# gregorgebhardt/gym-kilobots

Measured on AMD Instinct MI355X. Metric: kilobot-steps/sec, higher is better.
Workload: dtype f32

## Files before the change

### gym_kilobots_amd/csrc/kb_common.h

```cpp
#pragma once
#include <hip/hip_runtime.h>

#include <cmath>
#include <cstdio>
#include <cstring>
#include <type_traits>

#include "kilobots_hip.h"
#include "kb_launch.h"
#include "kb_exact.h"

namespace kb {

constexpr float B2_PI = 3.14159265359f;
constexpr float B2_LINEAR_SLOP = 0.005f;
constexpr float B2_POLYGON_RADIUS = 2.0f * B2_LINEAR_SLOP;
constexpr float B2_BAUMGARTE = 0.2f;
constexpr float B2_MAX_LINEAR_CORRECTION = 0.2f;
constexpr float B2_MAX_TRANSLATION = 2.0f;
constexpr float B2_MAX_TRANSLATION_SQ = B2_MAX_TRANSLATION * B2_MAX_TRANSLATION;
constexpr float B2_MAX_ROTATION = 0.5f * B2_PI;
constexpr float B2_MAX_ROTATION_SQ = B2_MAX_ROTATION * B2_MAX_ROTATION;
constexpr float B2_EPSILON = 1.19209290e-07f;
constexpr float B2_TOI_BAUMGARTE = 0.75f;
constexpr int B2_MAX_SUBSTEPS = 8;
constexpr float B2_TIME_TO_SLEEP = 0.5f;
constexpr float B2_LINEAR_SLEEP_TOL = 0.01f;
constexpr float B2_ANGULAR_SLEEP_TOL = 2.0f / 180.0f * B2_PI;
constexpr float WORLD_SCALE = 25.0f;

constexpr float CELL_SIZE = 0.875f;
constexpr int MAX_CELLS = 8192;

constexpr unsigned KEY_WALL = 0x10000u, KEY_OBJ = 0x20000u;
constexpr int WALL_CODE = 0xFFF0;
constexpr int OBJ_CODE = 0xFFE0;
constexpr int MAXOBJ = KB_MAX_OBJECTS;
constexpr unsigned short EMPTY16 = 0xFFFFu;

#ifndef KB_KREG
#define KB_KREG 2
#endif
constexpr int MAX_BUCKETS = MAX_WAVES * BK_PER_WAVE;
constexpr int GIANT_ISLAND = 256;
constexpr int BIG_ISLAND = 16;
constexpr int KREG = KB_KREG;
#ifndef KB_NSOLVE_DIV
#define KB_NSOLVE_DIV 1
#endif
#ifndef KB_KREG_BINS
#define KB_KREG_BINS (2 * KB_NSOLVE_DIV)
#endif

enum { M_NCON = 0, M_TOTAL = 1, M_ANY = 2, M_STATUS = 3, M_MAXISL = 4, M_PROF = 5, M_XTRA = 6, M_XFILL = 7, M_WCNT = 8, M_WAKE = 32 , M_WFILL = 8 + MAX_WAVES, M_COUNT = 8 + 2 * MAX_WAVES };
static_assert(M_COUNT <= 64, "misc area");

struct Params {
    kb_buffers buf;
    const float *actions;
    const float *light_action;
    int N, NP, NB, M, E, S, gw, gh, ncell, cap, capL, n_substeps, flags, drive_mode, light_type, vel_iters, pos_iters;
    int solver_mode, toi_walls;
    float xmin, ymin, xmax, ymax, inv_cell, r_bot, im_bot, kl_bot, ka_bot, h;
    float light_radius, light_lo[2], light_hi[2], act_lo[2], act_hi[2];
    int lcount, ladim, lkind[KB_MAX_LIGHTS];
    float lradius[KB_MAX_LIGHTS], lmaxv[KB_MAX_LIGHTS];
    float llo[KB_MAX_LIGHTS][2], lhi[KB_MAX_LIGHTS][2], lalo[KB_MAX_LIGHTS][2], lahi[KB_MAX_LIGHTS][2];
    float kl_obj, ka_obj;
    float otab[KB_MAX_OBJECTS][OT_WORDS_C];
    float obody[KB_MAX_OBJECTS][BT_WORDS_C];
    int F;
    float mu_oo, mu_ow;
    int nmc;
    int lds_total;
    int nhead, hmask;
    int allow_sleep;
    float im_mode[5];
    int botlaw_off;
    int islmin_off;
    int sense_s;
    float sense_r2;
    float rr2, rw2, rw_tot;
    float toi_tt;
    float nm_bb, nm_wb;
    float y_bb, y_wb;
    int exact_div;
    const unsigned char *env_mask;
};


__device__ __forceinline__ void kb_sincosf(float xx, float &sn, float &cs) {
    const float DP1 = 0.78515625f, DP2 = 2.4187564849853515625e-4f, DP3 = 3.77489497744594108e-8f;
    const float FOPI = 1.27323954473516f;
    float x = fabsf(xx);
    int j = (int)(FOPI * x);
    float y = (float)j;
    if (j & 1) { j += 1; y += 1.0f; }
    j &= 7;
    float ssign = xx < 0.0f ? -1.0f : 1.0f, csign = 1.0f;
    if (j > 3) { ssign = -ssign; csign = -csign; j -= 4; }
    if (j > 1) csign = -csign;
    x = ((x - y * DP1) - y * DP2) - y * DP3;
    float z = x * x;
    float pc = ((2.443315711809948E-005f * z - 1.388731625493765E-003f) * z + 4.166664568298827E-002f) * z * z
               - 0.5f * z + 1.0f;
    float ps = ((-1.9515295891E-4f * z + 8.3321608736E-3f) * z - 1.6666654611E-1f) * z * x + x;
    if (j == 1 || j == 2) { sn = ssign * pc; cs = csign * ps; }
    else { sn = ssign * ps; cs = csign * pc; }
}

__device__ __forceinline__ void kb_light_circular(float sx, float sy, float lx, float ly, float R,
                                                  float &val, float &gx, float &gy) {
    float dx = -1.0f * (sx - lx), dy = -1.0f * (sy - ly);
    float n = sqrtf(dx * dx + dy * dy);
    float v = 1.0f - n / R;
    v = fmaxf(fminf(v, 1.0f), 0.0f);
    val = v * 255.0f;
    if (n > 0.0f) { dx = dx / n; dy = dy / n; }
    else { dx = 0.0f; dy = 0.0f; }
    if (n > R) { dx *= 0.0f; dy *= 0.0f; }
    gx = dx; gy = dy;
}

__device__ __forceinline__ void kb_light_single_step(const Params &p, const float *la, float h, float &lx, float &ly) {
    float ax = fminf(fmaxf(la[0], p.act_lo[0]), p.act_hi[0]);
    float ay = fminf(fmaxf(la[1], p.act_lo[1]), p.act_hi[1]);
    float nlx = lx + ax * h, nly = ly + ay * h;
    lx = fminf(fmaxf(nlx, p.light_lo[0]), p.light_hi[0]);
    ly = fminf(fmaxf(nly, p.light_lo[1]), p.light_hi[1]);
}
__device__ __forceinline__ void kb_light_general_step(const Params &p, const float *la, float h, float (&glx)[KB_MAX_LIGHTS],
                                                      float (&gly)[KB_MAX_LIGHTS], float (&glvx)[KB_MAX_LIGHTS], float (&glvy)[KB_MAX_LIGHTS]) {
    if (p.light_type == KB_LIGHT_GRADIENT) {
        const float pi = 3.14159265358979323846f;
        float ang = fminf(fmaxf(la[0], -2.0f * pi), 2.0f * pi);
        if (ang < -pi) ang += 2.0f * pi;
        if (ang > pi) ang -= 2.0f * pi;
        glx[0] = ang;
    } else {
#pragma unroll
        for (int i = 0; i < KB_MAX_LIGHTS; ++i) {
            if (i >= p.lcount) break;
            const float ax = fminf(fmaxf(la[2 * i + 0], p.lalo[i][0]), p.lahi[i][0]);
            const float ay = fminf(fmaxf(la[2 * i + 1], p.lalo[i][1]), p.lahi[i][1]);
            float nlx, nly;
            if (p.lkind[i] == KB_LIGHT_MOMENTUM) {
                float mvx = glvx[i] + ax * h, mvy = glvy[i] + ay * h;
                const float nv = sqrtf(mvx * mvx + mvy * mvy);
                if (nv > p.lmaxv[i]) { const float sc = p.lmaxv[i] / nv; mvx *= sc; mvy *= sc; }
                glvx[i] = mvx; glvy[i] = mvy;
                nlx = glx[i] + mvx * h; nly = gly[i] + mvy * h;
            } else {
                nlx = glx[i] + ax * h; nly = gly[i] + ay * h;
            }
            glx[i] = fminf(fmaxf(nlx, p.llo[i][0]), p.lhi[i][0]);
            gly[i] = fminf(fmaxf(nly, p.llo[i][1]), p.lhi[i][1]);
        }
    }
}
__device__ __forceinline__ void kb_light_general_sense(const Params &p, const float (&glx)[KB_MAX_LIGHTS], const float (&gly)[KB_MAX_LIGHTS],
                                                       float sx, float sy, float &val, float &gx, float &gy) {
    if (p.light_type == KB_LIGHT_GRADIENT) {
        float s_, c_;
        kb_sincosf(glx[0], s_, c_);
        val = c_ * sx + s_ * sy; gx = c_; gy = s_;
        return;
    }
    float vsum = 0.0f, vbest = 0.0f, bgx = 0.0f, bgy = 0.0f;
#pragma unroll
    for (int i = 0; i < KB_MAX_LIGHTS; ++i) {
        if (i >= p.lcount) break;
        float v, x, y;
        kb_light_circular(sx, sy, glx[i], gly[i], p.lradius[i], v, x, y);
        vsum = i == 0 ? v : vsum + v;
        if (i == 0 || v > vbest) { vbest = v; bgx = x; bgy = y; }
    }
    val = vsum; gx = bgx; gy = bgy;
}

__device__ __forceinline__ void kb_motor_law(int ml, int mr, float th, float h, float &vx, float &vy, float &w) {
    const float max_lin = 0.01f, max_ang = 0.5f * 3.14159265358979323846f;
    float s, c;
    kb_sincosf(th, s, c);
    if (ml && mr) {
        float lin = (float)(mr + ml) / 510.0f * max_lin;
        vx = (s * lin) * WORLD_SCALE; vy = (c * lin) * WORLD_SCALE;
        w = (float)(mr - ml) / 510.0f * max_ang;
    } else if (mr || ml) {
        float av, lx, ly = -0.009f;
        if (mr) { av = (float)mr / 255.0f * max_ang; lx = -0.013f; }
        else { av = -(float)ml / 255.0f * max_ang; lx = 0.013f; }
        float ds, dc;
        kb_sincosf(av * h, ds, dc);
        float tx = lx - (dc * lx - ds * ly), ty = ly - (ds * lx + dc * ly);
        tx *= WORLD_SCALE; ty *= WORLD_SCALE;
        float wx = c * tx - s * ty, wy = s * tx + c * ty;
        wx = wx / WORLD_SCALE / h; wy = wy / WORLD_SCALE / h;
        vx = wx * WORLD_SCALE; vy = wy * WORLD_SCALE; w = av;
    } else {
        vx = 0.0f; vy = 0.0f; w = 0.0f;
    }
}

__device__ __forceinline__ float kb_clampf(float a, float lo, float hi) { return fmaxf(lo, fminf(a, hi)); }

__device__ __forceinline__ void wave_sync() {
    __builtin_amdgcn_fence(__ATOMIC_RELEASE, "wavefront");
    __builtin_amdgcn_wave_barrier();
    __builtin_amdgcn_fence(__ATOMIC_ACQUIRE, "wavefront");
}

template <bool DS_ATOMIC = false>
__device__ __forceinline__ unsigned lds_load_relaxed(const unsigned *p_) {
    if constexpr (DS_ATOMIC) return atomicOr(const_cast<unsigned *>(p_), 0u);
    else return *reinterpret_cast<const volatile unsigned *>(p_);
}

__device__ __forceinline__ void lds_barrier() {
    asm volatile("s_waitcnt lgkmcnt(0)\n\ts_barrier" ::: "memory");
}

#define KB_DPP(v, ctrl, rows) __builtin_amdgcn_update_dpp(0, (int)(v), ctrl, rows, 0xf, true)
__device__ __forceinline__ unsigned wave_or(unsigned v) {
    v |= (unsigned)KB_DPP(v, 0x111, 0xf);
    v |= (unsigned)KB_DPP(v, 0x112, 0xf);
    v |= (unsigned)KB_DPP(v, 0x114, 0xf);
    v |= (unsigned)KB_DPP(v, 0x118, 0xf);
    v |= (unsigned)KB_DPP(v, 0x142, 0xa);
    v |= (unsigned)KB_DPP(v, 0x143, 0xc);
    return (unsigned)__builtin_amdgcn_readlane((int)v, 63);
}
__device__ __forceinline__ unsigned wave_umax(unsigned v) {
    v = max(v, (unsigned)KB_DPP(v, 0x111, 0xf));
    v = max(v, (unsigned)KB_DPP(v, 0x112, 0xf));
    v = max(v, (unsigned)KB_DPP(v, 0x114, 0xf));
    v = max(v, (unsigned)KB_DPP(v, 0x118, 0xf));
    v = max(v, (unsigned)KB_DPP(v, 0x142, 0xa));
    v = max(v, (unsigned)KB_DPP(v, 0x143, 0xc));
    return (unsigned)__builtin_amdgcn_readlane((int)v, 63);
}
__device__ __forceinline__ unsigned wave_incl_scan(unsigned v) {
    v += (unsigned)KB_DPP(v, 0x111, 0xf);
    v += (unsigned)KB_DPP(v, 0x112, 0xf);
    v += (unsigned)KB_DPP(v, 0x114, 0xf);
    v += (unsigned)KB_DPP(v, 0x118, 0xf);
    v += (unsigned)KB_DPP(v, 0x142, 0xa);
    v += (unsigned)KB_DPP(v, 0x143, 0xc);
    return v;
}

template <class AR>
__device__ __forceinline__ void wall_geom(const AR &p, int wl, float x, float y, float &dist, float &nx, float &ny) {
    switch (wl) {
    case 0: nx = 1.0f; ny = 0.0f; dist = x - p.xmin; break;
    case 1: nx = 0.0f; ny = 1.0f; dist = y - p.ymin; break;
    case 2: nx = -1.0f; ny = 0.0f; dist = p.xmax - x; break;
    default: nx = 0.0f; ny = -1.0f; dist = p.ymax - y; break;
    }
}

#ifdef KB_PROFILE
#define KB_PROF(k) misc[24 + (k)]
#define KB_STAMP(ph) do { if (tid == 0) { const unsigned t_ = (unsigned)clock64(); atomicAdd(&KB_PROF(ph), t_ - prof_t); prof_t = t_; } } while (0)
#define KB_STAMP_PRE(ph) do { if (tid == 0) { atomicAdd(&KB_PROF(ph), (unsigned)clock64() - prof_t); } } while (0)
#else
#define KB_STAMP(ph) do { } while (0)
#define KB_STAMP_PRE(ph) do { } while (0)
#endif

template <class AR>
__device__ __forceinline__ bool kb_toi_wall(const AR &p, int wl, float R, float x0, float y0, float x1, float y1, float &tout) {
    const float total = R + B2_POLYGON_RADIUS;
    const float target = fmaxf(B2_LINEAR_SLOP, total - 3.0f * B2_LINEAR_SLOP);
    const float tol = 0.25f * B2_LINEAR_SLOP;
    float nx, ny;
    auto dist_at = [&](float t) __attribute__((always_inline)) -> float {
        float dv;
        wall_geom(p, wl, (1.0f - t) * x0 + t * x1, (1.0f - t) * y0 + t * y1, dv, nx, ny);
        return dv;
    };
    float t1 = 0.0f;
    for (int iter = 0; iter < 20; ++iter) {
        const float dist = dist_at(t1);
        if (fabsf(dist) <= 0.0f) return false;
        if (fabsf(dist) < target + tol) { tout = t1; return true; }
        float t2 = 1.0f;
        for (int push = 0; push < 8; ++push) {
            float s2 = dist_at(t2);
            if (s2 > target + tol) return false;
            if (s2 > target - tol) { t1 = t2; break; }
            float s1 = dist_at(t1);
            if (s1 < target - tol) return false;
            if (s1 <= target + tol) { tout = t1; return true; }
            float a1 = t1, a2 = t2;
            for (int root = 0; root < 50; ++root) {
                const float t = (root & 1) ? a1 + (target - s1) * (a2 - a1) / (s2 - s1) : 0.5f * (a1 + a2);
                const float sv = dist_at(t);
                if (fabsf(sv - target) < tol) { t2 = t; break; }
                if (sv > target) { a1 = t; s1 = sv; } else { a2 = t; s2 = sv; }
            }
        }
    }
    return false;
}

template <class AR>
__device__ __forceinline__ bool kb_toi_no_event(const AR &p, int wl, float tt, float x0, float y0, float x1, float y1) {
    float d0, d1, nx, ny;
    wall_geom(p, wl, (1.0f - 0.0f) * x0 + 0.0f * x1, (1.0f - 0.0f) * y0 + 0.0f * y1, d0, nx, ny);
    wall_geom(p, wl, (1.0f - 1.0f) * x0 + 1.0f * x1, (1.0f - 1.0f) * y0 + 1.0f * y1, d1, nx, ny);
    return fabsf(d0) <= 0.0f || (!(fabsf(d0) < tt) && d1 > tt);
}

__device__ __forceinline__ void kb_toi_walls_body(const Params &p, float R, float im, float x0, float y0, float a0,
                                                  float &x, float &y, float &a, float &vx, float &vy, float &w) {
    const float h = p.h;
    const float total = R + B2_POLYGON_RADIUS;
    {
        const float m0 = fminf(fminf(x0 - p.xmin, p.xmax - x0), fminf(y0 - p.ymin, p.ymax - y0));
        const float m1 = fminf(fminf(x - p.xmin, p.xmax - x), fminf(y - p.ymin, p.ymax - y));
        if (m0 > total && m1 > total) return;
    }
    float alpha0 = 0.0f;
    float c0x = x0, c0y = y0, ca0 = a0, cx = x, cy = y, ca = a;
    for (int ev = 0; ev < B2_MAX_SUBSTEPS; ++ev) {
        float minAlpha = 1.0f;
#pragma unroll
        for (int wl = 0; wl < 4; ++wl) {
            float t;
            float alpha = 1.0f;
            if (kb_toi_wall(p, wl, R, c0x, c0y, cx, cy, t)) alpha = fminf(alpha0 + (1.0f - alpha0) * t, 1.0f);
            if (alpha < minAlpha) minAlpha = alpha;
        }
        if (1.0f - 10.0f * B2_EPSILON < minAlpha) break;
        const float beta = (minAlpha - alpha0) / (1.0f - alpha0);
        c0x += beta * (cx - c0x); c0y += beta * (cy - c0y); ca0 += beta * (ca - ca0);
        alpha0 = minAlpha;
        cx = c0x; cy = c0y; ca = ca0;
        bool touch[4];
        float wnx[4], wny[4];
#pragma unroll
        for (int wl = 0; wl < 4; ++wl) {
            float dist;
            wall_geom(p, wl, cx, cy, dist, wnx[wl], wny[wl]);
            touch[wl] = !(dist * dist > total * total);
            if (dist < 0.0f) { wnx[wl] = -wnx[wl]; wny[wl] = -wny[wl]; }
        }
        for (int it = 0; it < 20; ++it) {
            float minSep = 0.0f;
#pragma unroll
            for (int wl = 0; wl < 4; ++wl) {
                if (!touch[wl]) continue;
                float dist, bx, by;
                wall_geom(p, wl, cx, cy, dist, bx, by);
// ... 234 lines not shown
```

### gym_kilobots_amd/csrc/kb_regsolve_bins.inc

```
{
    constexpr int KRB = KB_KREG_BINS;
    const bool solving = (int)__builtin_amdgcn_readfirstlane(wave) < nsolve;
    unsigned ra[KRB], rb[KRB], rm[KRB];
    float racc[KRB], rnx[KRB], rny[KRB];
    const unsigned WOFF = 8u * (unsigned)(NB - 5);
    char *const velB = reinterpret_cast<char *>(vel), *const posB = reinterpret_cast<char *>(pos);
#define RB_WALL(j) (ra[j] >= WOFF)
#define RB_WALLIDX(j) ((int)((ra[j] - WOFF) >> 3))
#define RB_VEL(off) (*reinterpret_cast<float2 *>(velB + (off)))
#define RB_POS(off) (*reinterpret_cast<float2 *>(posB + (off)))
#define RB_C(j) ((int)(rm[j] & 0xFFFu))
#define RB_DEPTH(j) ((int)((rm[j] >> 12) & 0x1FFu))
#define RB_FLIP(j) (((rm[j] >> 21) & 1u) != 0u)
#define RB_ISL(j) ((int)(rm[j] >> 22))
#pragma unroll
    for (int j = 0; j < KRB; ++j) { ra[j] = 0u; rb[j] = 0u; rm[j] = 0u; racc[j] = 0.0f; rnx[j] = 1.0f; rny[j] = 0.0f; }
    unsigned long long slotLevels[KRB];
    int dlo[KRB], dhi[KRB];
#pragma unroll
    for (int j = 0; j < KRB; ++j) { slotLevels[j] = 0ull; dlo[j] = 1; dhi[j] = 0; }
    int maxD = 0;
    unsigned mycnt = 0;
    const float nm_bb = p.nm_bb, nm_wb = p.nm_wb;
#ifdef KB_SOLVER_PRIO
    __builtin_amdgcn_s_setprio(KB_SOLVER_PRIO);
#endif
    if (solving) {
        mycnt = misc[M_WCNT + wave];
        const unsigned mybase = misc[M_WFILL + wave] - mycnt;
        unsigned lk[KRB];
        unsigned lp[KRB];
        int rdepth[KRB];
        unsigned klo[KRB], khi[KRB];
#define RB_A(j) ((int)(lp[j] & 0xFFFFu))
#define RB_B(j) ((int)(lp[j] >> 16))
        {
            unsigned c_[KRB], inf_[KRB];
            bool v_[KRB], awake_[KRB];
#pragma unroll
            for (int j = 0; j < KRB; ++j) {
                const unsigned idx = lane + 64u * j;
                v_[j] = idx < mycnt;
                c_[j] = lOrder[v_[j] ? mybase + idx : 0u];
            }
#pragma unroll
            for (int j = 0; j < KRB; ++j) {
                c_[j] = v_[j] ? c_[j] : 0u;
                lp[j] = lPair[c_[j]]; inf_[j] = lInfo[c_[j]];
            }
#pragma unroll
            for (int j = 0; j < KRB; ++j) { lp[j] = v_[j] ? lp[j] : 0u; awake_[j] = true; }
            if (SLEEP) {
                unsigned root_[KRB];
#pragma unroll
                for (int j = 0; j < KRB; ++j) root_[j] = parent[lp[j] >> 16];
#pragma unroll
                for (int j = 0; j < KRB; ++j) awake_[j] = active[root_[j]] != 0;
            }
#pragma unroll
            for (int j = 0; j < KRB; ++j) {
                const unsigned cls = inf_[j] & 0x7Fu, r = (inf_[j] >> 8) & 0xFFu;
                unsigned key = cls * RK + (r < RK - 1 ? r : RK - 1);
                const bool on = v_[j] && awake_[j];
                if (!on) key = 63u;
                const unsigned bit = on ? 1u << (key & 31u) : 0u;
                klo[j] = key < 32u ? bit : 0u; khi[j] = key < 32u ? 0u : bit;
                if (on && r >= RK - 1) atomicMax(&bkMaxRank[wave * NUM_CLS + cls], r);
                lk[j] = v_[j] ? (key | (r << 8) | (c_[j] << 16) | 0x80000000u) : 0u;
                rdepth[j] = 0;
            }
        }
        unsigned long long keymask = 0ull, restmask = 0ull;
        {
            unsigned mlo = 0, mhi = 0, rlo = 0, rhi = 0;
#pragma unroll
            for (int j = 0; j < KRB; ++j) { mlo |= klo[j]; mhi |= khi[j]; if (j > 0) { rlo |= klo[j]; rhi |= khi[j]; } }
            mlo = wave_or(mlo); mhi = wave_or(mhi);
            keymask = ((unsigned long long)mhi << 32) | mlo;
            if (mycnt > 64u) { rlo = wave_or(rlo); rhi = wave_or(rhi); restmask = ((unsigned long long)rhi << 32) | rlo; }
        }
        wave_sync();
#ifdef KB_PROFILE
        if (tid == 0) { atomicAdd(&KB_PROF(8), (unsigned)__popcll(keymask)); atomicAdd(&KB_PROF(11), 1u); }
#endif
        KB_STAMP_PRE(19);
        unsigned *bodyDepth = islCnt;
        {
            char *const bdB = reinterpret_cast<char *>(bodyDepth);
#define RB_BD(off) (*reinterpret_cast<unsigned *>(bdB + (off)))
            unsigned rc[KRB], ia4[KRB], ib4[KRB];
#pragma unroll
            for (int j = 0; j < KRB; ++j) {
                const unsigned key = lk[j] & 63u, r = (lk[j] >> 8) & 0xFFu;
                const bool on = (lk[j] >> 31) != 0u && key != 63u;
                rc[j] = on ? ((key % RK) == RK - 1 ? (key | (r << 6)) : key) : 0xFFFFFFFFu;
                ib4[j] = 4u * (unsigned)RB_B(j);
                ia4[j] = RB_A(j) < WALL_CODE ? 4u * (unsigned)RB_A(j) : ib4[j];
            }
            const unsigned mrow = bkMaxRank[wave * NUM_CLS + min((int)lane, NUM_CLS - 1)];
            for (unsigned long long m_ = keymask; m_; m_ &= m_ - 1) {
                const unsigned key_ = (unsigned)__builtin_ctzll(m_);
                const bool rest_ = ((restmask >> key_) & 1ull) != 0ull;
                auto depth_round = [&](unsigned code_) __attribute__((always_inline)) {
#pragma unroll
                    for (int j = 0; j < KRB; ++j) {
                        if (j == 0 || rest_) {
                            if (rc[j] == code_) {
                                const unsigned d = max(RB_BD(ia4[j]), RB_BD(ib4[j])) + 1u;
                                rdepth[j] = (int)d;
                                RB_BD(ib4[j]) = d;
                                RB_BD(ia4[j]) = d;
                            }
                        }
                    }
                    wave_sync();
                };
                if ((key_ % RK) < RK - 1) depth_round(key_);
                else {
                    const unsigned maxr_ = (unsigned)__builtin_amdgcn_readlane((int)mrow, (int)(key_ / RK));
                    for (unsigned r_ = RK - 1; r_ <= maxr_; ++r_) depth_round(key_ | (r_ << 6));
                }
            }
#undef RB_BD
        }
#pragma unroll
        for (int j = 0; j < KRB; ++j) maxD = max(maxD, rdepth[j]);
        maxD = (int)wave_umax((unsigned)maxD);
        KB_STAMP_PRE(20);
        if (mycnt > 64u) {
            unsigned at[KRB];
#pragma unroll
            for (int j = 0; j < KRB; ++j) at[j] = 0u;
            unsigned base_ = 0;
            for (int d_ = SLEEP ? 0 : 1; d_ <= maxD; ++d_) {
#pragma unroll
                for (int j = 0; j < KRB; ++j) {
                    const bool is = (lk[j] >> 31) && rdepth[j] == d_;
                    const unsigned long long m_ = __ballot(is);
                    const unsigned mine = __builtin_amdgcn_mbcnt_hi((unsigned)(m_ >> 32), __builtin_amdgcn_mbcnt_lo((unsigned)m_, base_));
                    at[j] = is ? mine : at[j];
                    base_ += (unsigned)__popcll(m_);
                }
            }
#pragma unroll
            for (int j = 0; j < KRB; ++j)
                if (lk[j] >> 31) {
                    lOrder[mybase + at[j]] = (unsigned short)((lk[j] >> 16) & 0xFFFu);
                    lCbk[mybase + at[j]] = (unsigned short)rdepth[j];
                }
            wave_sync();
            unsigned short o_[KRB], l_[KRB];
#pragma unroll
            for (int j = 0; j < KRB; ++j) {
                const unsigned i_ = mybase + ((lk[j] >> 31) ? lane + 64u * j : 0u);
                o_[j] = lOrder[i_]; l_[j] = lCbk[i_];
            }
#pragma unroll
            for (int j = 0; j < KRB; ++j) {
                const bool v_ = (lk[j] >> 31) != 0u;
                lk[j] = v_ ? ((lk[j] & 0x8000FFFFu) | ((unsigned)o_[j] << 16)) : lk[j];
                rdepth[j] = v_ ? (int)l_[j] : rdepth[j];
            }
        }
        KB_STAMP_PRE(21);
#pragma unroll
        for (int j = 0; j < KRB; ++j) {
            const unsigned long long mine = (lk[j] >> 31) ? 1ull << min(rdepth[j], 63) : 0ull;
            const unsigned lo = wave_or((unsigned)mine), hi = wave_or((unsigned)(mine >> 32));
            slotLevels[j] = ((unsigned long long)hi << 32) | (unsigned long long)lo;
            const unsigned long long lv = slotLevels[j] >> 1;
            dlo[j] = lv ? (int)__builtin_ctzll(lv) + 1 : 1;
            dhi[j] = lv ? ((lv >> 62) ? maxD : 64 - (int)__builtin_clzll(lv)) : 0;
        }
        {
            unsigned c_[KRB], pr_[KRB], inf_[KRB], root_[KRB];
            float acc_[KRB];
            float2 pa_[KRB], pb_[KRB];
            bool v_[KRB];
#pragma unroll
            for (int j = 0; j < KRB; ++j) {
                v_[j] = (lk[j] >> 31) != 0u;
                c_[j] = v_[j] ? (lk[j] >> 16) & 0xFFFu : 0u;
                pr_[j] = lPair[c_[j]]; inf_[j] = lInfo[c_[j]]; acc_[j] = lAcc[c_[j]];
            }
#pragma unroll
            for (int j = 0; j < KRB; ++j) {
                pr_[j] = v_[j] ? pr_[j] : 0u;
                const int a = (int)(pr_[j] & 0xFFFFu), b = (int)(pr_[j] >> 16);
                pa_[j] = pos[a >= WALL_CODE ? b : a]; pb_[j] = pos[b]; root_[j] = parent[b];
            }
            bool pairOn[KRB];
            float dx[KRB], dy[KRB], dd[KRB], wnx[KRB], wny[KRB];
            bool ieee = false;
#pragma unroll
            for (int j = 0; j < KRB; ++j) {
                const int a = (int)(pr_[j] & 0xFFFFu), b = (int)(pr_[j] >> 16);
                const bool wallA = a >= WALL_CODE, flip = (inf_[j] & 0x80u) != 0u;
                ra[j] = wallA ? WOFF + 8u * (unsigned)(a - WALL_CODE) : 8u * (unsigned)a;
                rb[j] = 8u * (unsigned)b;
                racc[j] = v_[j] ? acc_[j] : 0.0f;
                rm[j] = v_[j] ? (c_[j] | ((unsigned)rdepth[j] << 12) | (flip ? 1u << 21 : 0u) | (root_[j] << 22)) : 0u;
                float dist;
                wall_geom(p, wallA ? a - WALL_CODE : 0, pb_[j].x, pb_[j].y, dist, wnx[j], wny[j]);
                if (flip) { wnx[j] = -wnx[j]; wny[j] = -wny[j]; }
                dx[j] = pb_[j].x - pa_[j].x; dy[j] = pb_[j].y - pa_[j].y;
                dd[j] = dx[j] * dx[j] + dy[j] * dy[j];
                pairOn[j] = v_[j] && !wallA && dd[j] > B2_EPSILON * B2_EPSILON;
                ieee = ieee || (pairOn[j] && !kb_exact_guard(dd[j]));
                if (wallA) { rnx[j] = wnx[j]; rny[j] = wny[j]; } else { rnx[j] = 1.0f; rny[j] = 0.0f; }
            }
            if (__builtin_expect(__builtin_amdgcn_ballot_w64(ieee) == 0ull, 1)) {
#pragma unroll
                for (int j = 0; j < KRB; ++j) {
                    const float len = kb_sqrt_refine(dd[j], __builtin_amdgcn_sqrtf(dd[j]), __builtin_amdgcn_rsqf(dd[j]));
                    const float inv = kb_rcp_refine(len, __builtin_amdgcn_rcpf(len));
                    if (pairOn[j]) { rnx[j] = dx[j] * inv; rny[j] = dy[j] * inv; }
                }
            } else {
#pragma unroll
                for (int j = 0; j < KRB; ++j) {
                    const float len = sqrtf(dd[j]);
                    const float inv = 1.0f / len;
                    if (pairOn[j]) { rnx[j] = dx[j] * inv; rny[j] = dy[j] * inv; }
                }
            }
        }
#undef RB_A
#undef RB_B
#ifdef KB_PROFILE
        if (lane == 0) atomicMax(&misc[M_PROF], (unsigned)maxD);
        if (tid == 0) atomicAdd(&KB_PROF(M_PROF_DEPTH), (unsigned)maxD);
        {
            unsigned rounds_ = 0;
#pragma unroll
            for (int j = 0; j < KRB; ++j) rounds_ += dhi[j] >= dlo[j] ? (unsigned)(dhi[j] - dlo[j] + 1) : 0u;
            if (lane == 0) { if (mycnt > 64u) atomicAdd(&KB_PROF(36), 16u); atomicMax(&KB_PROF(38), rounds_); }
            if (tid == 0) atomicAdd(&KB_PROF(39), 16u * rounds_);
        }
        KB_STAMP(7);
#endif
    }
    KB_ABLATE_EXIT(9);
#define RB_ON(j) (RB_DEPTH(j) == d_)
    if (solving) {
#pragma unroll
        for (int j = 0; j < KRB; ++j) {
            for (int d_ = dlo[j]; d_ <= dhi[j]; ++d_) {
                if (RB_ON(j)) {
                    const float2 va = RB_VEL(ra[j]), vb = RB_VEL(rb[j]);
                    const float Px = racc[j] * rnx[j], Py = racc[j] * rny[j];
                    const float ima = RB_WALL(j) ? 0.0f : p.im_bot;
                    RB_VEL(ra[j]) = make_float2(va.x - ima * Px, va.y - ima * Py);
                    RB_VEL(rb[j]) = make_float2(vb.x + p.im_bot * Px, vb.y + p.im_bot * Py);
                }
                wave_sync();
            }
        }
        KB_STAMP_PRE(29);
    }
    KB_ABLATE_EXIT(10);
    if (solving) {
        for (int it = 0; it < p.vel_iters; ++it) {
#pragma unroll
            for (int j = 0; j < KRB; ++j) {
                for (int d_ = dlo[j]; d_ <= dhi[j]; ++d_) {
                    if (RB_ON(j)) {
                        const float2 va = RB_VEL(ra[j]), vb = RB_VEL(rb[j]);
                        const bool wallA = RB_WALL(j);
                        const float nx = rnx[j], ny = rny[j];
                        const float ima = wallA ? 0.0f : p.im_bot, imb = p.im_bot;
                        const float dvx = vb.x - va.x, dvy = vb.y - va.y;
                        const float vn = dvx * nx + dvy * ny;
                        float lambda = -((wallA ? nm_wb : nm_bb) * vn);
                        const float accOld = racc[j];
                        const float newimp = fmaxf(accOld + lambda, 0.0f);
                        lambda = newimp - accOld;
                        racc[j] = newimp;
                        const float Px = lambda * nx, Py = lambda * ny;
                        RB_VEL(ra[j]) = make_float2(va.x - ima * Px, va.y - ima * Py);
                        RB_VEL(rb[j]) = make_float2(vb.x + imb * Px, vb.y + imb * Py);
                    }
                    wave_sync();
                }
            }
        }
        KB_STAMP_PRE(30);
    }
    KB_STAMP(4);
    KB_RETID();
    KB_ABLATE_EXIT(11);
    if (solving) {
#pragma unroll
        for (int j = 0; j < KRB; ++j)
            if (lane + 64u * j < mycnt) lAcc[RB_C(j)] = racc[j];
    }
    {
        const unsigned char unsolved = (unsigned char)(p.pos_iters <= 0 ? 1 : 0);
        char *const sxB = reinterpret_cast<char *>(startX), *const syB = reinterpret_cast<char *>(startY);
        auto integrate_xy = [&](const unsigned off8, const float2 v0, const float2 p0) __attribute__((always_inline)) {
            float vxx = v0.x, vyy = v0.y;
            *reinterpret_cast<float *>(sxB + (off8 >> 1)) = p0.x; *reinterpret_cast<float *>(syB + (off8 >> 1)) = p0.y;
            const float tx = h * vxx, ty = h * vyy;
            if (tx * tx + ty * ty > B2_MAX_TRANSLATION_SQ) {
                const float ratio = B2_MAX_TRANSLATION / sqrtf(tx * tx + ty * ty);
                vxx *= ratio; vyy *= ratio;
            }
            RB_POS(off8) = make_float2(p0.x + h * vxx, p0.y + h * vyy);
            RB_VEL(off8) = make_float2(vxx, vyy);
        };
        bool intA[KRB], intB[KRB], own[BPT];
        {
            unsigned dA[KRB], dB[KRB], mk[BPT];
            const char *const bdB = reinterpret_cast<const char *>(islCnt);
#pragma unroll
            for (int j = 0; j < KRB; ++j) {
                dA[j] = *reinterpret_cast<const unsigned *>(bdB + ((RB_WALL(j) ? rb[j] : ra[j]) >> 1));
                dB[j] = *reinterpret_cast<const unsigned *>(bdB + (rb[j] >> 1));
            }
#pragma unroll
            for (int q = 0; q < BPT; ++q) mk[q] = intMark[(unsigned)ms[q] & 31u];
#pragma unroll
            for (int j = 0; j < KRB; ++j) {
                const unsigned d = (unsigned)RB_DEPTH(j);
                intA[j] = solving && d != 0u && !RB_WALL(j) && dA[j] == d;
                intB[j] = solving && d != 0u && dB[j] == d;
            }
#pragma unroll
            for (int q = 0; q < BPT; ++q) {
                own[q] = tid + q * nt < N && ((mk[q] >> ((unsigned)ms[q] >> 5)) & 1u) == 0u;
            }
        }
        wave_sync();
        static_assert(KRB == BPT, "a register slot and a kilobot of the owner thread share a trip");
#pragma unroll
        for (int j = 0; j < KRB; ++j) {
            const unsigned oo = 8u * (unsigned)ms[j];
            const float2 vO = RB_VEL(oo), pO = RB_POS(oo);
            const unsigned char aO = SLEEP ? active[ms[j]] : (unsigned char)1;
            if (j == 0 || mycnt > 64u) {
                const float2 vA = RB_VEL(ra[j]), vB = RB_VEL(rb[j]), pA = RB_POS(ra[j]), pB = RB_POS(rb[j]);
                if (intA[j]) {
                    integrate_xy(ra[j], vA, pA);
                    if (SLEEP) islWave[ra[j] >> 3] = (unsigned char)(2 | unsolved);
                }
                if (intB[j]) {
                    integrate_xy(rb[j], vB, pB);
                    if (SLEEP) islWave[rb[j] >> 3] = (unsigned char)(2 | unsolved);
                }
            }
            if (own[j]) {
                integrate_xy(oo, vO, pO);
                if (SLEEP) islWave[ms[j]] = (unsigned char)((aO ? 2 : 0) | unsolved);
            }
            float ww = bw[j];
            const float rot = h * ww;
            if (rot * rot > B2_MAX_ROTATION_SQ) {
                const float ratio = B2_MAX_ROTATION / fabsf(rot);
                ww *= ratio;
            }
            th[j] += h * ww;
            bw[j] = ww;
        }
    }
    wave_sync();
    KB_STAMP(5);
    KB_ABLATE_EXIT(12);
    if (solving) {
        for (int it = 0; it < p.pos_iters; ++it) {
            unsigned char *act = active + (it & 1) * NB, *nxt = active + ((it + 1) & 1) * NB;
            bool viol = false;
            bool ron[KRB];
#pragma unroll
            for (int j = 0; j < KRB; ++j) ron[j] = (lane + 64u * j < mycnt) && act[RB_ISL(j)] != 0;
#pragma unroll
            for (int j = 0; j < KRB; ++j) {
                for (int d_ = dlo[j]; d_ <= dhi[j]; ++d_) {
                    if (ron[j] && RB_ON(j)) {
                    const bool wallA = RB_WALL(j);
                    const int isl = RB_ISL(j);
                    float nx, ny, sep;
                    const float ima = wallA ? 0.0f : p.im_bot, imb = p.im_bot;
                    const float2 pb = RB_POS(rb[j]);
                    const float bx = pb.x, by = pb.y;
                    float axx = 0.0f, ayy = 0.0f;
                    if (wallA) {
                        float dist, wx, wy;
                        wall_geom(p, RB_WALLIDX(j), bx, by, dist, wx, wy);
                        nx = RB_FLIP(j) ? -wx : wx; ny = RB_FLIP(j) ? -wy : wy;
                        const float along = RB_FLIP(j) ? -dist : dist;
                        sep = along - B2_POLYGON_RADIUS - p.r_bot;
                    } else {
                        const float2 pa = RB_POS(ra[j]);
                        axx = pa.x; ayy = pa.y;
                        const float dx = bx - axx, dy = by - ayy;
                        const float dd = dx * dx + dy * dy;
                        if (__builtin_expect(__builtin_amdgcn_ballot_w64(!kb_exact_guard(dd)) == 0ull, 1)) {
                            const float len = kb_sqrt_refine(dd, __builtin_amdgcn_sqrtf(dd), __builtin_amdgcn_rsqf(dd));
                            const float inv = kb_rcp_refine(len, __builtin_amdgcn_rcpf(len));
                            nx = dx * inv; ny = dy * inv;
                        } else {
                            const float len = sqrtf(dd);
                            nx = dx; ny = dy;
                            if (!(len < B2_EPSILON)) { const float inv = 1.0f / len; nx = dx * inv; ny = dy * inv; }
                        }
                        sep = (dx * nx + dy * ny) - p.r_bot - p.r_bot;
                    }
                    if (sep < -3.0f * B2_LINEAR_SLOP) { nxt[isl] = 1; viol = true; if (SLEEP && it == p.pos_iters - 1) islWave[isl] = 3; }
                    const float C = kb_clampf(B2_BAUMGARTE * (sep + B2_LINEAR_SLOP), -B2_MAX_LINEAR_CORRECTION, 0.0f);
                    const float K = ima + imb;
                    const float imp = __builtin_expect(p.exact_div, 1) ? kb_div_const(-C, K, wallA ? p.y_wb : p.y_bb) : (K > 0.0f ? -C / K : 0.0f);
                    const float Px = imp * nx, Py = imp * ny;
                    if (!wallA) RB_POS(ra[j]) = make_float2(axx - ima * Px, ayy - ima * Py);
                    RB_POS(rb[j]) = make_float2(bx + imb * Px, by + imb * Py);
                    }
                    wave_sync();
                }
            }
#ifdef KB_PROFILE
            if (tid == 0) atomicAdd(&KB_PROF(10), 1u);
#endif
            if (!__any(viol)) break;
#pragma unroll
            for (int j = 0; j < KRB; ++j) if (lane + 64u * j < mycnt) act[RB_ISL(j)] = 0;
            wave_sync();
        }
        KB_STAMP_PRE(24);
    }
#ifdef KB_SOLVER_PRIO
    __builtin_amdgcn_s_setprio(0);
#endif
#undef RB_WALL
#undef RB_WALLIDX
#undef RB_VEL
#undef RB_POS
#undef RB_C
#undef RB_DEPTH
#undef RB_FLIP
#undef RB_ISL
#undef RB_ON
}
```

Measured before the change: 17.30 billion.

## Add single-slot fused setup path merging depth coloring with warm-start impulses

```diff
diff --git a/gym_kilobots_amd/csrc/kb_common.h b/gym_kilobots_amd/csrc/kb_common.h
--- a/gym_kilobots_amd/csrc/kb_common.h
+++ b/gym_kilobots_amd/csrc/kb_common.h
@@ -50,6 +50,9 @@
 #endif
 #ifndef KB_KREG_BINS
 #define KB_KREG_BINS (2 * KB_NSOLVE_DIV)
+#endif
+#ifndef KB_SETUP_FUSED
+#define KB_SETUP_FUSED 2
 #endif
 
 enum { M_NCON = 0, M_TOTAL = 1, M_ANY = 2, M_STATUS = 3, M_MAXISL = 4, M_PROF = 5, M_XTRA = 6, M_XFILL = 7, M_WCNT = 8, M_WAKE = 32 , M_WFILL = 8 + MAX_WAVES, M_COUNT = 8 + 2 * MAX_WAVES };
diff --git a/gym_kilobots_amd/csrc/kb_regsolve_bins.inc b/gym_kilobots_amd/csrc/kb_regsolve_bins.inc
--- a/gym_kilobots_amd/csrc/kb_regsolve_bins.inc
+++ b/gym_kilobots_amd/csrc/kb_regsolve_bins.inc
@@ -21,6 +21,7 @@
     for (int j = 0; j < KRB; ++j) { slotLevels[j] = 0ull; dlo[j] = 1; dhi[j] = 0; }
     int maxD = 0;
     unsigned mycnt = 0;
+    bool twoSlot = false;
     const float nm_bb = p.nm_bb, nm_wb = p.nm_wb;
 #ifdef KB_SOLVER_PRIO
     __builtin_amdgcn_s_setprio(KB_SOLVER_PRIO);
@@ -28,205 +29,298 @@
     if (solving) {
         mycnt = misc[M_WCNT + wave];
         const unsigned mybase = misc[M_WFILL + wave] - mycnt;
-        unsigned lk[KRB];
-        unsigned lp[KRB];
-        int rdepth[KRB];
-        unsigned klo[KRB], khi[KRB];
+        twoSlot = KB_SETUP_FUSED == 0 || (unsigned)__builtin_amdgcn_readfirstlane((int)mycnt) > 64u;
+        if (twoSlot) {
+            unsigned lk[KRB];
+            unsigned lp[KRB];
+            int rdepth[KRB];
+            unsigned klo[KRB], khi[KRB];
 #define RB_A(j) ((int)(lp[j] & 0xFFFFu))
 #define RB_B(j) ((int)(lp[j] >> 16))
-        {
-            unsigned c_[KRB], inf_[KRB];
-            bool v_[KRB], awake_[KRB];
-#pragma unroll
-            for (int j = 0; j < KRB; ++j) {
-                const unsigned idx = lane + 64u * j;
-                v_[j] = idx < mycnt;
-                c_[j] = lOrder[v_[j] ? mybase + idx : 0u];
-            }
-#pragma unroll
-            for (int j = 0; j < KRB; ++j) {
-                c_[j] = v_[j] ? c_[j] : 0u;
-                lp[j] = lPair[c_[j]]; inf_[j] = lInfo[c_[j]];
-            }
-#pragma unroll
-            for (int j = 0; j < KRB; ++j) { lp[j] = v_[j] ? lp[j] : 0u; awake_[j] = true; }
-            if (SLEEP) {
-                unsigned root_[KRB];
-#pragma unroll
-                for (int j = 0; j < KRB; ++j) root_[j] = parent[lp[j] >> 16];
-#pragma unroll
-                for (int j = 0; j < KRB; ++j) awake_[j] = active[root_[j]] != 0;
-            }
-#pragma unroll
-            for (int j = 0; j < KRB; ++j) {
-                const unsigned cls = inf_[j] & 0x7Fu, r = (inf_[j] >> 8) & 0xFFu;
-                unsigned key = cls * RK + (r < RK - 1 ? r : RK - 1);
-                const bool on = v_[j] && awake_[j];
-                if (!on) key = 63u;
-                const unsigned bit = on ? 1u << (key & 31u) : 0u;
-                klo[j] = key < 32u ? bit : 0u; khi[j] = key < 32u ? 0u : bit;
-                if (on && r >= RK - 1) atomicMax(&bkMaxRank[wave * NUM_CLS + cls], r);
-                lk[j] = v_[j] ? (key | (r << 8) | (c_[j] << 16) | 0x80000000u) : 0u;
-                rdepth[j] = 0;
-            }
-        }
-        unsigned long long keymask = 0ull, restmask = 0ull;
-        {
-            unsigned mlo = 0, mhi = 0, rlo = 0, rhi = 0;
-#pragma unroll
-            for (int j = 0; j < KRB; ++j) { mlo |= klo[j]; mhi |= khi[j]; if (j > 0) { rlo |= klo[j]; rhi |= khi[j]; } }
-            mlo = wave_or(mlo); mhi = wave_or(mhi);
-            keymask = ((unsigned long long)mhi << 32) | mlo;
-            if (mycnt > 64u) { rlo = wave_or(rlo); rhi = wave_or(rhi); restmask = ((unsigned long long)rhi << 32) | rlo; }
-        }
-        wave_sync();
+            {
+                unsigned c_[KRB], inf_[KRB];
+                bool v_[KRB], awake_[KRB];
+#pragma unroll
+                for (int j = 0; j < KRB; ++j) {
+                    const unsigned idx = lane + 64u * j;
+                    v_[j] = idx < mycnt;
+                    c_[j] = lOrder[v_[j] ? mybase + idx : 0u];
+                }
+#pragma unroll
+                for (int j = 0; j < KRB; ++j) {
+                    c_[j] = v_[j] ? c_[j] : 0u;
+                    lp[j] = lPair[c_[j]]; inf_[j] = lInfo[c_[j]];
+                }
+#pragma unroll
+                for (int j = 0; j < KRB; ++j) { lp[j] = v_[j] ? lp[j] : 0u; awake_[j] = true; }
+                if (SLEEP) {
+                    unsigned root_[KRB];
+#pragma unroll
+                    for (int j = 0; j < KRB; ++j) root_[j] = parent[lp[j] >> 16];
+#pragma unroll
+                    for (int j = 0; j < KRB; ++j) awake_[j] = active[root_[j]] != 0;
+                }
+#pragma unroll
+                for (int j = 0; j < KRB; ++j) {
+                    const unsigned cls = inf_[j] & 0x7Fu, r = (inf_[j] >> 8) & 0xFFu;
+                    unsigned key = cls * RK + (r < RK - 1 ? r : RK - 1);
+                    const bool on = v_[j] && awake_[j];
+                    if (!on) key = 63u;
+                    const unsigned bit = on ? 1u << (key & 31u) : 0u;
+                    klo[j] = key < 32u ? bit : 0u; khi[j] = key < 32u ? 0u : bit;
+                    if (on && r >= RK - 1) atomicMax(&bkMaxRank[wave * NUM_CLS + cls], r);
+                    lk[j] = v_[j] ? (key | (r << 8) | (c_[j] << 16) | 0x80000000u) : 0u;
+                    rdepth[j] = 0;
+                }
+            }
+            unsigned long long keymask = 0ull, restmask = 0ull;
+            {
+                unsigned mlo = 0, mhi = 0, rlo = 0, rhi = 0;
+#pragma unroll
+                for (int j = 0; j < KRB; ++j) { mlo |= klo[j]; mhi |= khi[j]; if (j > 0) { rlo |= klo[j]; rhi |= khi[j]; } }
+                mlo = wave_or(mlo); mhi = wave_or(mhi);
+                keymask = ((unsigned long long)mhi << 32) | mlo;
+                if (mycnt > 64u) { rlo = wave_or(rlo); rhi = wave_or(rhi); restmask = ((unsigned long long)rhi << 32) | rlo; }
+            }
+            wave_sync();
 #ifdef KB_PROFILE
-        if (tid == 0) { atomicAdd(&KB_PROF(8), (unsigned)__popcll(keymask)); atomicAdd(&KB_PROF(11), 1u); }
+            if (tid == 0) { atomicAdd(&KB_PROF(8), (unsigned)__popcll(keymask)); atomicAdd(&KB_PROF(11), 1u); }
 #endif
-        KB_STAMP_PRE(19);
-        unsigned *bodyDepth = islCnt;
-        {
-            char *const bdB = reinterpret_cast<char *>(bodyDepth);
+            KB_STAMP_PRE(19);
+            unsigned *bodyDepth = islCnt;
+            {
+                char *const bdB = reinterpret_cast<char *>(bodyDepth);
 #define RB_BD(off) (*reinterpret_cast<unsigned *>(bdB + (off)))
-            unsigned rc[KRB], ia4[KRB], ib4[KRB];
-#pragma unroll
-            for (int j = 0; j < KRB; ++j) {
-                const unsigned key = lk[j] & 63u, r = (lk[j] >> 8) & 0xFFu;
-                const bool on = (lk[j] >> 31) != 0u && key != 63u;
-                rc[j] = on ? ((key % RK) == RK - 1 ? (key | (r << 6)) : key) : 0xFFFFFFFFu;
-                ib4[j] = 4u * (unsigned)RB_B(j);
-                ia4[j] = RB_A(j) < WALL_CODE ? 4u * (unsigned)RB_A(j) : ib4[j];
-            }
-            const unsigned mrow = bkMaxRank[wave * NUM_CLS + min((int)lane, NUM_CLS - 1)];
-            for (unsigned long long m_ = keymask; m_; m_ &= m_ - 1) {
-                const unsigned key_ = (unsigned)__builtin_ctzll(m_);
-                const bool rest_ = ((restmask >> key_) & 1ull) != 0ull;
-                auto depth_round = [&](unsigned code_) __attribute__((always_inline)) {
-#pragma unroll
-                    for (int j = 0; j < KRB; ++j) {
-                        if (j == 0 || rest_) {
-                            if (rc[j] == code_) {
-                                const unsigned d = max(RB_BD(ia4[j]), RB_BD(ib4[j])) + 1u;
-                                rdepth[j] = (int)d;
-                                RB_BD(ib4[j]) = d;
-                                RB_BD(ia4[j]) = d;
+                unsigned rc[KRB], ia4[KRB], ib4[KRB];
+#pragma unroll
+                for (int j = 0; j < KRB; ++j) {
+                    const unsigned key = lk[j] & 63u, r = (lk[j] >> 8) & 0xFFu;
+                    const bool on = (lk[j] >> 31) != 0u && key != 63u;
+                    rc[j] = on ? ((key % RK) == RK - 1 ? (key | (r << 6)) : key) : 0xFFFFFFFFu;
+                    ib4[j] = 4u * (unsigned)RB_B(j);
+                    ia4[j] = RB_A(j) < WALL_CODE ? 4u * (unsigned)RB_A(j) : ib4[j];
+                }
+                const unsigned mrow = bkMaxRank[wave * NUM_CLS + min((int)lane, NUM_CLS - 1)];
+                for (unsigned long long m_ = keymask; m_; m_ &= m_ - 1) {
+                    const unsigned key_ = (unsigned)__builtin_ctzll(m_);
+                    const bool rest_ = ((restmask >> key_) & 1ull) != 0ull;
+                    auto depth_round = [&](unsigned code_) __attribute__((always_inline)) {
+#pragma unroll
+                        for (int j = 0; j < KRB; ++j) {
+                            if (j == 0 || rest_) {
+                                if (rc[j] == code_) {
+                                    const unsigned d = max(RB_BD(ia4[j]), RB_BD(ib4[j])) + 1u;
+                                    rdepth[j] = (int)d;
+                                    RB_BD(ib4[j]) = d;
+                                    RB_BD(ia4[j]) = d;
+                                }
                             }
                         }
-                    }
-                    wave_sync();
-                };
-                if ((key_ % RK) < RK - 1) depth_round(key_);
-                else {
-                    const unsigned maxr_ = (unsigned)__builtin_amdgcn_readlane((int)mrow, (int)(key_ / RK));
-                    for (unsigned r_ = RK - 1; r_ <= maxr_; ++r_) depth_round(key_ | (r_ << 6));
-                }
-            }
+                        wave_sync();
+                    };
+                    if ((key_ % RK) < RK - 1) depth_round(key_);
+                    else {
+                        const unsigned maxr_ = (unsigned)__builtin_amdgcn_readlane((int)mrow, (int)(key_ / RK));
+                        for (unsigned r_ = RK - 1; r_ <= maxr_; ++r_) depth_round(key_ | (r_ << 6));
+                    }
+                }
 #undef RB_BD
-        }
-#pragma unroll
-        for (int j = 0; j < KRB; ++j) maxD = max(maxD, rdepth[j]);
-        maxD = (int)wave_umax((unsigned)maxD);
-        KB_STAMP_PRE(20);
-        if (mycnt > 64u) {
-            unsigned at[KRB];
-#pragma unroll
-            for (int j = 0; j < KRB; ++j) at[j] = 0u;
-            unsigned base_ = 0;
-            for (int d_ = SLEEP ? 0 : 1; d_ <= maxD; ++d_) {
-#pragma unroll
-                for (int j = 0; j < KRB; ++j) {
-                    const bool is = (lk[j] >> 31) && rdepth[j] == d_;
-                    const unsigned long long m_ = __ballot(is);
-                    const unsigned mine = __builtin_amdgcn_mbcnt_hi((unsigned)(m_ >> 32), __builtin_amdgcn_mbcnt_lo((unsigned)m_, base_));
-                    at[j] = is ? mine : at[j];
-                    base_ += (unsigned)__popcll(m_);
-                }
-            }
-#pragma unroll
-            for (int j = 0; j < KRB; ++j)
-                if (lk[j] >> 31) {
-                    lOrder[mybase + at[j]] = (unsigned short)((lk[j] >> 16) & 0xFFFu);
-                    lCbk[mybase + at[j]] = (unsigned short)rdepth[j];
-                }
-            wave_sync();
-            unsigned short o_[KRB], l_[KRB];
+            }
+#pragma unroll
+            for (int j = 0; j < KRB; ++j) maxD = max(maxD, rdepth[j]);
+            maxD = (int)wave_umax((unsigned)maxD);
+            KB_STAMP_PRE(20);
+            if (mycnt > 64u) {
+                unsigned at[KRB];
+#pragma unroll
+                for (int j = 0; j < KRB; ++j) at[j] = 0u;
+                unsigned base_ = 0;
+                for (int d_ = SLEEP ? 0 : 1; d_ <= maxD; ++d_) {
+#pragma unroll
+                    for (int j = 0; j < KRB; ++j) {
+                        const bool is = (lk[j] >> 31) && rdepth[j] == d_;
+                        const unsigned long long m_ = __ballot(is);
+                        const unsigned mine = __builtin_amdgcn_mbcnt_hi((unsigned)(m_ >> 32), __builtin_amdgcn_mbcnt_lo((unsigned)m_, base_));
+                        at[j] = is ? mine : at[j];
+                        base_ += (unsigned)__popcll(m_);
+                    }
+                }
+#pragma unroll
+                for (int j = 0; j < KRB; ++j)
+                    if (lk[j] >> 31) {
+                        lOrder[mybase + at[j]] = (unsigned short)((lk[j] >> 16) & 0xFFFu);
+                        lCbk[mybase + at[j]] = (unsigned short)rdepth[j];
+                    }
+                wave_sync();
+                unsigned short o_[KRB], l_[KRB];
+#pragma unroll
+                for (int j = 0; j < KRB; ++j) {
+                    const unsigned i_ = mybase + ((lk[j] >> 31) ? lane + 64u * j : 0u);
+                    o_[j] = lOrder[i_]; l_[j] = lCbk[i_];
+                }
+#pragma unroll
+                for (int j = 0; j < KRB; ++j) {
+                    const bool v_ = (lk[j] >> 31) != 0u;
+                    lk[j] = v_ ? ((lk[j] & 0x8000FFFFu) | ((unsigned)o_[j] << 16)) : lk[j];
+                    rdepth[j] = v_ ? (int)l_[j] : rdepth[j];
+                }
+            }
+            KB_STAMP_PRE(21);
 #pragma unroll
             for (int j = 0; j < KRB; ++j) {
-                const unsigned i_ = mybase + ((lk[j] >> 31) ? lane + 64u * j : 0u);
-                o_[j] = lOrder[i_]; l_[j] = lCbk[i_];
-            }
-#pragma unroll
-            for (int j = 0; j < KRB; ++j) {
-                const bool v_ = (lk[j] >> 31) != 0u;
-                lk[j] = v_ ? ((lk[j] & 0x8000FFFFu) | ((unsigned)o_[j] << 16)) : lk[j];
-                rdepth[j] = v_ ? (int)l_[j] : rdepth[j];
-            }
-        }
-        KB_STAMP_PRE(21);
-#pragma unroll
-        for (int j = 0; j < KRB; ++j) {
-            const unsigned long long mine = (lk[j] >> 31) ? 1ull << min(rdepth[j], 63) : 0ull;
-            const unsigned lo = wave_or((unsigned)mine), hi = wave_or((unsigned)(mine >> 32));
-            slotLevels[j] = ((unsigned long long)hi << 32) | (unsigned long long)lo;
-            const unsigned long long lv = slotLevels[j] >> 1;
-            dlo[j] = lv ? (int)__builtin_ctzll(lv) + 1 : 1;
-            dhi[j] = lv ? ((lv >> 62) ? maxD : 64 - (int)__builtin_clzll(lv)) : 0;
-        }
-        {
-            unsigned c_[KRB], pr_[KRB], inf_[KRB], root_[KRB];
-            float acc_[KRB];
-            float2 pa_[KRB], pb_[KRB];
-            bool v_[KRB];
-#pragma unroll
-            for (int j = 0; j < KRB; ++j) {
-                v_[j] = (lk[j] >> 31) != 0u;
-                c_[j] = v_[j] ? (lk[j] >> 16) & 0xFFFu : 0u;
-                pr_[j] = lPair[c_[j]]; inf_[j] = lInfo[c_[j]]; acc_[j] = lAcc[c_[j]];
-            }
-#pragma unroll
-            for (int j = 0; j < KRB; ++j) {
-                pr_[j] = v_[j] ? pr_[j] : 0u;
-                const int a = (int)(pr_[j] & 0xFFFFu), b = (int)(pr_[j] >> 16);
-                pa_[j] = pos[a >= WALL_CODE ? b : a]; pb_[j] = pos[b]; root_[j] = parent[b];
-            }
-            bool pairOn[KRB];
-            float dx[KRB], dy[KRB], dd[KRB], wnx[KRB], wny[KRB];
-            bool ieee = false;
-#pragma unroll
-            for (int j = 0; j < KRB; ++j) {
-                const int a = (int)(pr_[j] & 0xFFFFu), b = (int)(pr_[j] >> 16);
-                const bool wallA = a >= WALL_CODE, flip = (inf_[j] & 0x80u) != 0u;
-                ra[j] = wallA ? WOFF + 8u * (unsigned)(a - WALL_CODE) : 8u * (unsigned)a;
-                rb[j] = 8u * (unsigned)b;
-                racc[j] = v_[j] ? acc_[j] : 0.0f;
-                rm[j] = v_[j] ? (c_[j] | ((unsigned)rdepth[j] << 12) | (flip ? 1u << 21 : 0u) | (root_[j] << 22)) : 0u;
-                float dist;
-                wall_geom(p, wallA ? a - WALL_CODE : 0, pb_[j].x, pb_[j].y, dist, wnx[j], wny[j]);
-                if (flip) { wnx[j] = -wnx[j]; wny[j] = -wny[j]; }
-                dx[j] = pb_[j].x - pa_[j].x; dy[j] = pb_[j].y - pa_[j].y;
-                dd[j] = dx[j] * dx[j] + dy[j] * dy[j];
-                pairOn[j] = v_[j] && !wallA && dd[j] > B2_EPSILON * B2_EPSILON;
-                ieee = ieee || (pairOn[j] && !kb_exact_guard(dd[j]));
-                if (wallA) { rnx[j] = wnx[j]; rny[j] = wny[j]; } else { rnx[j] = 1.0f; rny[j] = 0.0f; }
-            }
-            if (__builtin_expect(__builtin_amdgcn_ballot_w64(ieee) == 0ull, 1)) {
-#pragma unroll
-                for (int j = 0; j < KRB; ++j) {
-                    const float len = kb_sqrt_refine(dd[j], __builtin_amdgcn_sqrtf(dd[j]), __builtin_amdgcn_rsqf(dd[j]));
-                    const float inv = kb_rcp_refine(len, __builtin_amdgcn_rcpf(len));
-                    if (pairOn[j]) { rnx[j] = dx[j] * inv; rny[j] = dy[j] * inv; }
-                }
-            } else {
-#pragma unroll
-                for (int j = 0; j < KRB; ++j) {
-                    const float len = sqrtf(dd[j]);
-                    const float inv = 1.0f / len;
-                    if (pairOn[j]) { rnx[j] = dx[j] * inv; rny[j] = dy[j] * inv; }
-                }
-            }
-        }
+                const unsigned long long mine = (lk[j] >> 31) ? 1ull << min(rdepth[j], 63) : 0ull;
+                const unsigned lo = wave_or((unsigned)mine), hi = wave_or((unsigned)(mine >> 32));
+                slotLevels[j] = ((unsigned long long)hi << 32) | (unsigned long long)lo;
+                const unsigned long long lv = slotLevels[j] >> 1;
+                dlo[j] = lv ? (int)__builtin_ctzll(lv) + 1 : 1;
+                dhi[j] = lv ? ((lv >> 62) ? maxD : 64 - (int)__builtin_clzll(lv)) : 0;
+            }
+            {
+                unsigned c_[KRB], pr_[KRB], inf_[KRB], root_[KRB];
+                float acc_[KRB];
+                float2 pa_[KRB], pb_[KRB];
+                bool v_[KRB];
+#pragma unroll
+                for (int j = 0; j < KRB; ++j) {
+                    v_[j] = (lk[j] >> 31) != 0u;
+                    c_[j] = v_[j] ? (lk[j] >> 16) & 0xFFFu : 0u;
+                    pr_[j] = lPair[c_[j]]; inf_[j] = lInfo[c_[j]]; acc_[j] = lAcc[c_[j]];
+                }
+#pragma unroll
+                for (int j = 0; j < KRB; ++j) {
+                    pr_[j] = v_[j] ? pr_[j] : 0u;
+                    const int a = (int)(pr_[j] & 0xFFFFu), b = (int)(pr_[j] >> 16);
+                    pa_[j] = pos[a >= WALL_CODE ? b : a]; pb_[j] = pos[b]; root_[j] = parent[b];
+                }
+                bool pairOn[KRB];
+                float dx[KRB], dy[KRB], dd[KRB], wnx[KRB], wny[KRB];
+                bool ieee = false;
+#pragma unroll
+                for (int j = 0; j < KRB; ++j) {
+                    const int a = (int)(pr_[j] & 0xFFFFu), b = (int)(pr_[j] >> 16);
+                    const bool wallA = a >= WALL_CODE, flip = (inf_[j] & 0x80u) != 0u;
+                    ra[j] = wallA ? WOFF + 8u * (unsigned)(a - WALL_CODE) : 8u * (unsigned)a;
+                    rb[j] = 8u * (unsigned)b;
+                    racc[j] = v_[j] ? acc_[j] : 0.0f;
+                    rm[j] = v_[j] ? (c_[j] | ((unsigned)rdepth[j] << 12) | (flip ? 1u << 21 : 0u) | (root_[j] << 22)) : 0u;
+                    float dist;
+                    wall_geom(p, wallA ? a - WALL_CODE : 0, pb_[j].x, pb_[j].y, dist, wnx[j], wny[j]);
+                    if (flip) { wnx[j] = -wnx[j]; wny[j] = -wny[j]; }
+                    dx[j] = pb_[j].x - pa_[j].x; dy[j] = pb_[j].y - pa_[j].y;
+                    dd[j] = dx[j] * dx[j] + dy[j] * dy[j];
+                    pairOn[j] = v_[j] && !wallA && dd[j] > B2_EPSILON * B2_EPSILON;
+                    ieee = ieee || (pairOn[j] && !kb_exact_guard(dd[j]));
+                    if (wallA) { rnx[j] = wnx[j]; rny[j] = wny[j]; } else { rnx[j] = 1.0f; rny[j] = 0.0f; }
+                }
+                if (__builtin_expect(__builtin_amdgcn_ballot_w64(ieee) == 0ull, 1)) {
+#pragma unroll
+                    for (int j = 0; j < KRB; ++j) {
+                        const float len = kb_sqrt_refine(dd[j], __builtin_amdgcn_sqrtf(dd[j]), __builtin_amdgcn_rsqf(dd[j]));
+                        const float inv = kb_rcp_refine(len, __builtin_amdgcn_rcpf(len));
+                        if (pairOn[j]) { rnx[j] = dx[j] * inv; rny[j] = dy[j] * inv; }
+                    }
+                } else {
+#pragma unroll
+                    for (int j = 0; j < KRB; ++j) {
+                        const float len = sqrtf(dd[j]);
+                        const float inv = 1.0f / len;
+                        if (pairOn[j]) { rnx[j] = dx[j] * inv; rny[j] = dy[j] * inv; }
+                    }
+                }
+            }
 #undef RB_A
 #undef RB_B
+        } else {
+            const bool v_ = lane < mycnt;
+            unsigned c_ = lOrder[v_ ? mybase + lane : 0u];
+            c_ = v_ ? c_ : 0u;
+            unsigned pr_ = lPair[c_];
+            const unsigned inf_ = lInfo[c_];
+            const float acc_ = lAcc[c_];
+            pr_ = v_ ? pr_ : 0u;
+            const int a = (int)(pr_ & 0xFFFFu), b = (int)(pr_ >> 16);
+            const bool wallA = a >= WALL_CODE, flip = (inf_ & 0x80u) != 0u;
+            const float2 pa_ = pos[wallA ? b : a], pb_ = pos[b];
+            const unsigned root_ = parent[b];
+            bool awake_ = true;
+            if (SLEEP) awake_ = active[root_] != 0;
+            const unsigned cls = inf_ & 0x7Fu, r = (inf_ >> 8) & 0xFFu;
+            const unsigned key = cls * RK + (r < RK - 1 ? r : RK - 1);
+            const bool on = v_ && awake_;
+            if (on && r >= RK - 1) atomicMax(&bkMaxRank[wave * NUM_CLS + cls], r);
+            const unsigned rc = on ? (r >= RK - 1 ? (key | (r << 6)) : key) : 0xFFFFFFFFu;
+            const unsigned bit = on ? 1u << (key & 31u) : 0u;
+            const unsigned long long keymask = ((unsigned long long)wave_or(key < 32u ? 0u : bit) << 32) | wave_or(key < 32u ? bit : 0u);
+            ra[0] = wallA ? WOFF + 8u * (unsigned)(a - WALL_CODE) : 8u * (unsigned)a;
+            rb[0] = 8u * (unsigned)b;
+            racc[0] = v_ ? acc_ : 0.0f;
+            rm[0] = v_ ? (c_ | (flip ? 1u << 21 : 0u) | (root_ << 22)) : 0u;
+            {
+                float dist, wnx, wny;
+                wall_geom(p, wallA ? a - WALL_CODE : 0, pb_.x, pb_.y, dist, wnx, wny);
+                if (flip) { wnx = -wnx; wny = -wny; }
+                const float dx = pb_.x - pa_.x, dy = pb_.y - pa_.y;
+                const float dd = dx * dx + dy * dy;
+                const bool pairOn = v_ && !wallA && dd > B2_EPSILON * B2_EPSILON;
+                if (wallA) { rnx[0] = wnx; rny[0] = wny; } else { rnx[0] = 1.0f; rny[0] = 0.0f; }
+                if (__builtin_expect(__builtin_amdgcn_ballot_w64(pairOn && !kb_exact_guard(dd)) == 0ull, 1)) {
+                    const float len = kb_sqrt_refine(dd, __builtin_amdgcn_sqrtf(dd), __builtin_amdgcn_rsqf(dd));
+                    const float inv = kb_rcp_refine(len, __builtin_amdgcn_rcpf(len));
+                    if (pairOn) { rnx[0] = dx * inv; rny[0] = dy * inv; }
+                } else {
+                    const float len = sqrtf(dd);
+                    const float inv = 1.0f / len;
+                    if (pairOn) { rnx[0] = dx * inv; rny[0] = dy * inv; }
+                }
+            }
+            wave_sync();
+#ifdef KB_PROFILE
+            if (tid == 0) { atomicAdd(&KB_PROF(8), (unsigned)__popcll(keymask)); atomicAdd(&KB_PROF(11), 1u); }
+#endif
+            KB_STAMP_PRE(19);
+            {
+                char *const bdB = reinterpret_cast<char *>(islCnt);
+#define RB_BD(off) (*reinterpret_cast<unsigned *>(bdB + (off)))
+                const unsigned ib4 = rb[0] >> 1, ia4 = wallA ? ib4 : ra[0] >> 1;
+                const float Px = racc[0] * rnx[0], Py = racc[0] * rny[0];
+                const float ima = wallA ? 0.0f : p.im_bot;
+                const float dax = ima * Px, day = ima * Py, dbx = p.im_bot * Px, dby = p.im_bot * Py;
+                const unsigned mrow = bkMaxRank[wave * NUM_CLS + min((int)lane, NUM_CLS - 1)];
+                unsigned depth_ = 0;
+                for (unsigned long long m_ = keymask; m_; m_ &= m_ - 1) {
+                    const unsigned key_ = (unsigned)__builtin_ctzll(m_);
+                    auto depth_round = [&](unsigned code_) __attribute__((always_inline)) {
+                        if (rc == code_) {
+                            const unsigned d = max(RB_BD(ia4), RB_BD(ib4)) + 1u;
+                            if (KB_SETUP_FUSED >= 2) {
+                                const float2 va = RB_VEL(ra[0]), vb = RB_VEL(rb[0]);
+                                RB_VEL(ra[0]) = make_float2(va.x - dax, va.y - day);
+                                RB_VEL(rb[0]) = make_float2(vb.x + dbx, vb.y + dby);
+                            }
+                            depth_ = d;
+                            RB_BD(ib4) = d;
+                            RB_BD(ia4) = d;
+                        }
+                        wave_sync();
+                    };
+                    if ((key_ % RK) < RK - 1) depth_round(key_);
+                    else {
+                        const unsigned maxr_ = (unsigned)__builtin_amdgcn_readlane((int)mrow, (int)(key_ / RK));
+                        for (unsigned r_ = RK - 1; r_ <= maxr_; ++r_) depth_round(key_ | (r_ << 6));
+                    }
+                }
+#undef RB_BD
+                rm[0] |= depth_ << 12;
+                maxD = (int)wave_umax(depth_);
+                KB_STAMP_PRE(20);
+                KB_STAMP_PRE(21);
+                const unsigned long long mine = v_ ? 1ull << min(depth_, 63u) : 0ull;
+                slotLevels[0] = ((unsigned long long)wave_or((unsigned)(mine >> 32)) << 32) | (unsigned long long)wave_or((unsigned)mine);
+                const unsigned long long lv = slotLevels[0] >> 1;
+                dlo[0] = lv ? (int)__builtin_ctzll(lv) + 1 : 1;
+                dhi[0] = lv ? ((lv >> 62) ? maxD : 64 - (int)__builtin_clzll(lv)) : 0;
+            }
+        }
 #ifdef KB_PROFILE
         if (lane == 0) atomicMax(&misc[M_PROF], (unsigned)maxD);
         if (tid == 0) atomicAdd(&KB_PROF(M_PROF_DEPTH), (unsigned)maxD);
@@ -243,17 +337,19 @@
     KB_ABLATE_EXIT(9);
 #define RB_ON(j) (RB_DEPTH(j) == d_)
     if (solving) {
-#pragma unroll
-        for (int j = 0; j < KRB; ++j) {
-            for (int d_ = dlo[j]; d_ <= dhi[j]; ++d_) {
-                if (RB_ON(j)) {
-                    const float2 va = RB_VEL(ra[j]), vb = RB_VEL(rb[j]);
-                    const float Px = racc[j] * rnx[j], Py = racc[j] * rny[j];
-                    const float ima = RB_WALL(j) ? 0.0f : p.im_bot;
-                    RB_VEL(ra[j]) = make_float2(va.x - ima * Px, va.y - ima * Py);
-                    RB_VEL(rb[j]) = make_float2(vb.x + p.im_bot * Px, vb.y + p.im_bot * Py);
-                }
-                wave_sync();
+        if (twoSlot || KB_SETUP_FUSED < 2) {
+#pragma unroll
+            for (int j = 0; j < KRB; ++j) {
+                for (int d_ = dlo[j]; d_ <= dhi[j]; ++d_) {
+                    if (RB_ON(j)) {
+                        const float2 va = RB_VEL(ra[j]), vb = RB_VEL(rb[j]);
+                        const float Px = racc[j] * rnx[j], Py = racc[j] * rny[j];
+                        const float ima = RB_WALL(j) ? 0.0f : p.im_bot;
+                        RB_VEL(ra[j]) = make_float2(va.x - ima * Px, va.y - ima * Py);
+                        RB_VEL(rb[j]) = make_float2(vb.x + p.im_bot * Px, vb.y + p.im_bot * Py);
+                    }
+                    wave_sync();
+                }
             }
         }
         KB_STAMP_PRE(29);
```

Result: faster. 17.52 billion, median of 6 (+1.3%).
